# XuyangBai/D3Feat

Measured on NVIDIA H100. Metric: points/sec through KPFCNN encoder, higher is better.
Workload: dtype f32

## Files before the change

### d3feat_b200/csrc/ops.cuh

```cuda
#pragma once
#include "common.cuh"

namespace d3f {

struct Epilogue {
  const float* rowscale;
  const float* bn_scale;
  const float* bn_shift;
  const float* bias;
  const float* residual;
  float leaky_alpha;
  const int* row_map;
  const int* m_dev = nullptr;
  int m_off = 0;
};
int gemm_f32(const float* A, const float* B, float* C, int M, int N, int K, const Epilogue& ep, cudaStream_t stream);

size_t tc_packed_floats(int K, int N);
int tc_padded_n(int N);
int tc_pack_weight(const float* W, int K, int N, float* packed, cudaStream_t stream);
bool tc_gemm_supported(const float* A, int K);
int tc_gemm(const float* A, const float* Bp, float* C, int M, int N, int K, const Epilogue& ep, cudaStream_t stream,
            float* split_ws = nullptr, const float* A2 = nullptr, int K1 = 0);
int tc_gemm_splits(int M, int N, int K);
size_t tc_gemm_split_ws_floats(int M, int N, int K);

int launch_batch_start(const int* len, int B, int* start, cudaStream_t stream);
int bbox_device(const float* pts, int N, float* out_bbox, cudaStream_t stream);
size_t grid_subsample_workspace_bytes(int N, int B);
int grid_subsample(const float* pts, const int* batch_len, int B, int N, float dl, const float* feats, int fdim,
                   const int* classes, int ldim, const float* host_bbox, float* out_pts, float* out_feats,
                   int* out_classes, int* out_batch_len, int* out_M, void* workspace, size_t workspace_bytes,
                   cudaStream_t stream, const int* n_dev = nullptr, int out_capacity = -1, int* status = nullptr,
                   const int* start_pre = nullptr);

size_t voxel_down_sample_workspace_bytes(int N, int B);
int voxel_down_sample(const float* pts, const int* lengths, int B, int N, const int* n_dev, double voxel_size,
                      const float* host_bbox, float* out_pts, int* out_lengths, int* out_M, int out_capacity,
                      int* d_status, void* workspace, size_t workspace_bytes, cudaStream_t stream);

size_t radius_neighbors_workspace_bytes(int Ns, int B, float radius, const float* host_bbox);
int radius_neighbors_build(const float* supports, const int* s_batch_len, int B, int Ns, float radius,
                           const float* host_bbox, void* workspace, size_t workspace_bytes, cudaStream_t stream,
                           const int* ns_dev = nullptr, const int* s_start_pre = nullptr);
int radius_neighbors_count(const float* queries, const int* q_batch_len, int Nq, int B, int Ns, float radius,
                           const float* host_bbox, const void* workspace, int* counts, int* out_max,
                           cudaStream_t stream);
int radius_neighbors_order(const void* workspace, int Ns, int B, float radius, const float* host_bbox, int* out_order,
                           cudaStream_t stream);
int radius_neighbors_fill(const float* queries, const int* q_batch_len, int Nq, int B, int Ns, float radius,
                          const float* host_bbox, const void* workspace, int cols, int pad_value, int* out_idx,
                          cudaStream_t stream, const int* nq_dev = nullptr, const int* pad_dev = nullptr,
                          const int* q_start_pre = nullptr);
struct NbView;
int radius_neighbors_view(const void* workspace, int Ns, int B, float radius, const float* host_bbox, NbView* out);

size_t pyramid_workspace_bytes(int B, const d3f_pyramid_spec* spec, const int* capacity, const float* host_bbox);
int pyramid_build(const float* points, const int* lengths, int B, int N0, const d3f_pyramid_spec* spec,
                  const float* host_bbox, float* const* out_points, int* const* out_lengths,
                  int* const* out_neighbors, int* const* out_pools, int* const* out_upsamples, const int* capacity,
                  int* out_level_sizes, void* workspace, size_t workspace_bytes, cudaStream_t stream,
                  int* d_counts = nullptr, int* d_status = nullptr, const int* n0_dev = nullptr);

size_t kpconv_workspace_bytes(int Nq, int Ns, int H, int K, int Cin, int Cout);
int kpconv_forward_impl(bool deform, const float* q, const float* s, const int* idx, const float* feat,
                        const float* Kp, const float* offsets, const float* modulations, const float* W,
                        const float* W_packed, const int* query_order, int Nq,
                        int Ns, int H, int K, int Cin, int Cout, float extent, int influence, int mode, int normalize,
                        const float* bn_scale, const float* bn_shift, const float* bias, float leaky_alpha,
                        float* out, void* workspace, size_t workspace_bytes, cudaStream_t stream,
                        const int* nq_dev = nullptr, const int* ns_dev = nullptr);

bool kpconv_fused_supported(int Nq, int H, int K, int Cin, int Cout, int influence, int mode, const float* feat,
                            const float* W, const float* out, const int* query_order);
size_t kpconv_fused_workspace_bytes();
int kpconv_fused_forward(const float* q, const float4* s4, const int* idx, const float* feat, const float* Kp,
                         const float* W, float* w_img, int Nq, int Ns, int H, int Cout, float extent, int normalize,
                         const float* bn_scale, const float* bn_shift, const float* bias, float leaky_alpha, float* out,
                         cudaStream_t stream, const int* nq_dev = nullptr, const int* ns_dev = nullptr);

int ind_max_pool(const float* x, const int* inds, int N1, int N2, int H, int C, float* out, void* workspace,
                 size_t workspace_bytes, cudaStream_t stream, const int* n1_dev = nullptr, const int* n2_dev = nullptr);
int closest_pool(const float* x, const int* inds, int N1, int N2, int ld_inds, int C, float* out,
                 cudaStream_t stream, const int* n1_dev = nullptr, const int* n2_dev = nullptr);
int l2_normalize(const float* x, int N, int C, float eps, float* out, cudaStream_t stream, const int* n_dev = nullptr);
size_t detection_scores_workspace_bytes(int N, int B);
int detection_scores(const float* feats, const int* neighbors, const int* lengths, int B, int N, int H, int D,
                     float* out_scores, void* workspace, size_t workspace_bytes, cudaStream_t stream,
                     const int* n_dev = nullptr);
int affine_leaky(const float* x, int N, int C, const float* scale, const float* shift, const float* residual,
                 float alpha, float* out, cudaStream_t stream, const int* n_dev = nullptr);

size_t select_keypoints_workspace_bytes(int N, int B);
int select_keypoints(const float* scores, const int* lengths, int B, int N, int k, const float* points,
                     const float* descriptors, int D, int* out_order, int* out_index, int* out_count, float* out_points,
                     float* out_descriptors, float* out_scores, void* workspace, size_t workspace_bytes,
                     cudaStream_t stream, const int* n_dev = nullptr);

size_t match_descriptors_workspace_bytes(int k, int P);
int match_descriptors(const float* desc, const int* count, int B, int k, int D, const int* pairs, int P, int* nn_st,
                      float* sim_st, int* nn_ts, float* sim_ts, int* matches, int* n_matches, void* workspace,
                      size_t workspace_bytes, cudaStream_t stream);

size_t register_pairs_workspace_bytes(int L, int P, int max_iterations, int max_validation);
int register_pairs(const float* points, const int* count, int B, int k, const int* corr, const int* n_corr, int L,
                   const int* pairs, int P, int ransac_n, int max_iterations, int max_validation, double distance,
                   double edge_ratio, unsigned long long seed, double* pose, int* n_inliers, int* hypothesis,
                   int* n_validated, void* workspace, size_t workspace_bytes, cudaStream_t stream);

size_t icp_pairs_workspace_bytes(int N, int B, int P, double distance, const float* host_bbox);
int icp_pairs(const float* points, const int* lengths, int B, int N, const int* n_dev, const float* host_bbox,
              const int* pairs, int P, const double* init, double distance, int max_iterations,
              double relative_fitness, double relative_rmse, double* pose, double* fitness, double* inlier_rmse,
              int* n_corr, int* iterations, void* workspace, size_t workspace_bytes, cudaStream_t stream);

size_t evaluate_pairs_workspace_bytes(int P, int S);
int evaluate_pairs(const float* points, const int* count, int B, int k, const int* matches, const int* n_matches,
                   int L, const int* pairs, int P, const double* truth_pose, const double* truth_info,
                   const int* truth_flags, const double* const* poses, int S, const int* levels, int R,
                   double fmr_distance, double fmr_ratio, double repeat_distance, double err2, double rte_max,
                   double rre_max_deg, int* valid, int* n_match_inliers, double* inlier_ratio, int* fmr_hit,
                   int* n_repeated, double* repeatability, double* rte, double* rre_deg, double* rmse2, int* success,
                   int* recall_hit, double* totals, void* workspace, size_t workspace_bytes, cudaStream_t stream);

}
```

### d3feat_b200/csrc/tc_common.cuh

```cuda
#pragma once
#include "common.cuh"

namespace d3f {

__device__ __forceinline__ uint32_t smem_u32(const void* p) { return (uint32_t)__cvta_generic_to_shared(p); }

__device__ __forceinline__ void mbar_init(uint32_t bar, uint32_t count) {
  asm volatile("mbarrier.init.shared::cta.b64 [%0], %1;" ::"r"(bar), "r"(count) : "memory");
}
__device__ __forceinline__ void mbar_arrive(uint32_t bar) {
  asm volatile("mbarrier.arrive.shared::cta.b64 _, [%0];" ::"r"(bar) : "memory");
}
__device__ __forceinline__ void mbar_wait(uint32_t bar, uint32_t parity) {
  uint32_t ok;
  do {
    asm volatile(
        "{\n\t.reg .pred p;\n\t"
        "mbarrier.try_wait.parity.shared::cta.b64 p, [%1], %2;\n\t"
        "selp.u32 %0, 1, 0, p;\n\t}"
        : "=r"(ok)
        : "r"(bar), "r"(parity)
        : "memory");
  } while (!ok);
}
__device__ __forceinline__ void fence_proxy_async() { asm volatile("fence.proxy.async.shared::cta;" ::: "memory"); }

__device__ __forceinline__ uint64_t make_smem_desc(uint32_t saddr) {
  uint64_t d = 0;
  d |= (uint64_t)((saddr >> 4) & 0x3FFF);
  d |= (uint64_t)1 << 16;
  d |= (uint64_t)(1024 >> 4) << 32;
  d |= (uint64_t)1 << 62;
  return d;
}

__device__ __forceinline__ void wgmma_fence() { asm volatile("wgmma.fence.sync.aligned;" ::: "memory"); }
__device__ __forceinline__ void wgmma_commit() { asm volatile("wgmma.commit_group.sync.aligned;" ::: "memory"); }
template <int N>
__device__ __forceinline__ void wgmma_wait() { asm volatile("wgmma.wait_group.sync.aligned %0;" ::"n"(N) : "memory"); }
template <int R>
__device__ __forceinline__ void wgmma_reg_fence(float* d) {
#pragma unroll
  for (int i = 0; i < R; ++i) asm volatile("" : "+f"(d[i])::"memory");
}

template <int N>
__device__ __forceinline__ void wgmma_tf32(float* d, uint64_t adesc, uint64_t bdesc);
template <>
__device__ __forceinline__ void wgmma_tf32<32>(float* d, uint64_t adesc, uint64_t bdesc) {
  asm volatile(
      "{\n\t.reg .pred p;\n\tsetp.ne.b32 p, %18, 0;\n\t"
      "wgmma.mma_async.sync.aligned.m64n32k8.f32.tf32.tf32 "
      "{%0, %1, %2, %3, %4, %5, %6, %7, %8, %9, %10, %11, %12, %13, %14, %15}, %16, %17, p, 1, 1;\n\t}"
      : "+f"(d[0]), "+f"(d[1]), "+f"(d[2]), "+f"(d[3]), "+f"(d[4]), "+f"(d[5]), "+f"(d[6]), "+f"(d[7]), "+f"(d[8]), "+f"(d[9]), "+f"(d[10]), "+f"(d[11]), "+f"(d[12]), "+f"(d[13]), "+f"(d[14]), "+f"(d[15])
      : "l"(adesc), "l"(bdesc), "r"(1)
      : "memory");
}
template <>
__device__ __forceinline__ void wgmma_tf32<64>(float* d, uint64_t adesc, uint64_t bdesc) {
  asm volatile(
      "{\n\t.reg .pred p;\n\tsetp.ne.b32 p, %34, 0;\n\t"
      "wgmma.mma_async.sync.aligned.m64n64k8.f32.tf32.tf32 "
      "{%0, %1, %2, %3, %4, %5, %6, %7, %8, %9, %10, %11, %12, %13, %14, %15, %16, %17, %18, %19, %20, %21, %22, %23, %24, %25, %26, %27, %28, %29, %30, %31}, %32, %33, p, 1, 1;\n\t}"
      : "+f"(d[0]), "+f"(d[1]), "+f"(d[2]), "+f"(d[3]), "+f"(d[4]), "+f"(d[5]), "+f"(d[6]), "+f"(d[7]), "+f"(d[8]), "+f"(d[9]), "+f"(d[10]), "+f"(d[11]), "+f"(d[12]), "+f"(d[13]), "+f"(d[14]), "+f"(d[15]), "+f"(d[16]), "+f"(d[17]), "+f"(d[18]), "+f"(d[19]), "+f"(d[20]), "+f"(d[21]), "+f"(d[22]), "+f"(d[23]), "+f"(d[24]), "+f"(d[25]), "+f"(d[26]), "+f"(d[27]), "+f"(d[28]), "+f"(d[29]), "+f"(d[30]), "+f"(d[31])
      : "l"(adesc), "l"(bdesc), "r"(1)
      : "memory");
}
template <>
__device__ __forceinline__ void wgmma_tf32<96>(float* d, uint64_t adesc, uint64_t bdesc) {
  asm volatile(
      "{\n\t.reg .pred p;\n\tsetp.ne.b32 p, %50, 0;\n\t"
      "wgmma.mma_async.sync.aligned.m64n96k8.f32.tf32.tf32 "
      "{%0, %1, %2, %3, %4, %5, %6, %7, %8, %9, %10, %11, %12, %13, %14, %15, %16, %17, %18, %19, %20, %21, %22, %23, %24, %25, %26, %27, %28, %29, %30, %31, %32, %33, %34, %35, %36, %37, %38, %39, %40, %41, %42, %43, %44, %45, %46, %47}, %48, %49, p, 1, 1;\n\t}"
      : "+f"(d[0]), "+f"(d[1]), "+f"(d[2]), "+f"(d[3]), "+f"(d[4]), "+f"(d[5]), "+f"(d[6]), "+f"(d[7]), "+f"(d[8]), "+f"(d[9]), "+f"(d[10]), "+f"(d[11]), "+f"(d[12]), "+f"(d[13]), "+f"(d[14]), "+f"(d[15]), "+f"(d[16]), "+f"(d[17]), "+f"(d[18]), "+f"(d[19]), "+f"(d[20]), "+f"(d[21]), "+f"(d[22]), "+f"(d[23]), "+f"(d[24]), "+f"(d[25]), "+f"(d[26]), "+f"(d[27]), "+f"(d[28]), "+f"(d[29]), "+f"(d[30]), "+f"(d[31]), "+f"(d[32]), "+f"(d[33]), "+f"(d[34]), "+f"(d[35]), "+f"(d[36]), "+f"(d[37]), "+f"(d[38]), "+f"(d[39]), "+f"(d[40]), "+f"(d[41]), "+f"(d[42]), "+f"(d[43]), "+f"(d[44]), "+f"(d[45]), "+f"(d[46]), "+f"(d[47])
      : "l"(adesc), "l"(bdesc), "r"(1)
      : "memory");
}
template <>
__device__ __forceinline__ void wgmma_tf32<128>(float* d, uint64_t adesc, uint64_t bdesc) {
  asm volatile(
      "{\n\t.reg .pred p;\n\tsetp.ne.b32 p, %66, 0;\n\t"
      "wgmma.mma_async.sync.aligned.m64n128k8.f32.tf32.tf32 "
      "{%0, %1, %2, %3, %4, %5, %6, %7, %8, %9, %10, %11, %12, %13, %14, %15, %16, %17, %18, %19, %20, %21, %22, %23, %24, %25, %26, %27, %28, %29, %30, %31, %32, %33, %34, %35, %36, %37, %38, %39, %40, %41, %42, %43, %44, %45, %46, %47, %48, %49, %50, %51, %52, %53, %54, %55, %56, %57, %58, %59, %60, %61, %62, %63}, %64, %65, p, 1, 1;\n\t}"
      : "+f"(d[0]), "+f"(d[1]), "+f"(d[2]), "+f"(d[3]), "+f"(d[4]), "+f"(d[5]), "+f"(d[6]), "+f"(d[7]), "+f"(d[8]), "+f"(d[9]), "+f"(d[10]), "+f"(d[11]), "+f"(d[12]), "+f"(d[13]), "+f"(d[14]), "+f"(d[15]), "+f"(d[16]), "+f"(d[17]), "+f"(d[18]), "+f"(d[19]), "+f"(d[20]), "+f"(d[21]), "+f"(d[22]), "+f"(d[23]), "+f"(d[24]), "+f"(d[25]), "+f"(d[26]), "+f"(d[27]), "+f"(d[28]), "+f"(d[29]), "+f"(d[30]), "+f"(d[31]), "+f"(d[32]), "+f"(d[33]), "+f"(d[34]), "+f"(d[35]), "+f"(d[36]), "+f"(d[37]), "+f"(d[38]), "+f"(d[39]), "+f"(d[40]), "+f"(d[41]), "+f"(d[42]), "+f"(d[43]), "+f"(d[44]), "+f"(d[45]), "+f"(d[46]), "+f"(d[47]), "+f"(d[48]), "+f"(d[49]), "+f"(d[50]), "+f"(d[51]), "+f"(d[52]), "+f"(d[53]), "+f"(d[54]), "+f"(d[55]), "+f"(d[56]), "+f"(d[57]), "+f"(d[58]), "+f"(d[59]), "+f"(d[60]), "+f"(d[61]), "+f"(d[62]), "+f"(d[63])
      : "l"(adesc), "l"(bdesc), "r"(1)
      : "memory");
}

template <int N>
__device__ __forceinline__ void wgmma_tf32_rs(float* d, const uint32_t* a, uint64_t bdesc);
template <>
__device__ __forceinline__ void wgmma_tf32_rs<32>(float* d, const uint32_t* a, uint64_t bdesc) {
  asm volatile(
      "{\n\t.reg .pred p;\n\tsetp.ne.b32 p, %21, 0;\n\t"
      "wgmma.mma_async.sync.aligned.m64n32k8.f32.tf32.tf32 "
      "{%0, %1, %2, %3, %4, %5, %6, %7, %8, %9, %10, %11, %12, %13, %14, %15}, {%16, %17, %18, %19}, %20, p, 1, 1;\n\t}"
      : "+f"(d[0]), "+f"(d[1]), "+f"(d[2]), "+f"(d[3]), "+f"(d[4]), "+f"(d[5]), "+f"(d[6]), "+f"(d[7]), "+f"(d[8]), "+f"(d[9]), "+f"(d[10]), "+f"(d[11]), "+f"(d[12]), "+f"(d[13]), "+f"(d[14]), "+f"(d[15])
      : "r"(a[0]), "r"(a[1]), "r"(a[2]), "r"(a[3]), "l"(bdesc), "r"(1)
      : "memory");
}
template <>
__device__ __forceinline__ void wgmma_tf32_rs<64>(float* d, const uint32_t* a, uint64_t bdesc) {
  asm volatile(
      "{\n\t.reg .pred p;\n\tsetp.ne.b32 p, %37, 0;\n\t"
      "wgmma.mma_async.sync.aligned.m64n64k8.f32.tf32.tf32 "
      "{%0, %1, %2, %3, %4, %5, %6, %7, %8, %9, %10, %11, %12, %13, %14, %15, %16, %17, %18, %19, %20, %21, %22, %23, %24, %25, %26, %27, %28, %29, %30, %31}, {%32, %33, %34, %35}, %36, p, 1, 1;\n\t}"
      : "+f"(d[0]), "+f"(d[1]), "+f"(d[2]), "+f"(d[3]), "+f"(d[4]), "+f"(d[5]), "+f"(d[6]), "+f"(d[7]), "+f"(d[8]), "+f"(d[9]), "+f"(d[10]), "+f"(d[11]), "+f"(d[12]), "+f"(d[13]), "+f"(d[14]), "+f"(d[15]), "+f"(d[16]), "+f"(d[17]), "+f"(d[18]), "+f"(d[19]), "+f"(d[20]), "+f"(d[21]), "+f"(d[22]), "+f"(d[23]), "+f"(d[24]), "+f"(d[25]), "+f"(d[26]), "+f"(d[27]), "+f"(d[28]), "+f"(d[29]), "+f"(d[30]), "+f"(d[31])
      : "r"(a[0]), "r"(a[1]), "r"(a[2]), "r"(a[3]), "l"(bdesc), "r"(1)
      : "memory");
}
template <>
__device__ __forceinline__ void wgmma_tf32_rs<128>(float* d, const uint32_t* a, uint64_t bdesc) {
  asm volatile(
      "{\n\t.reg .pred p;\n\tsetp.ne.b32 p, %69, 0;\n\t"
      "wgmma.mma_async.sync.aligned.m64n128k8.f32.tf32.tf32 "
      "{%0, %1, %2, %3, %4, %5, %6, %7, %8, %9, %10, %11, %12, %13, %14, %15, %16, %17, %18, %19, %20, %21, %22, %23, %24, %25, %26, %27, %28, %29, %30, %31, %32, %33, %34, %35, %36, %37, %38, %39, %40, %41, %42, %43, %44, %45, %46, %47, %48, %49, %50, %51, %52, %53, %54, %55, %56, %57, %58, %59, %60, %61, %62, %63}, {%64, %65, %66, %67}, %68, p, 1, 1;\n\t}"
      : "+f"(d[0]), "+f"(d[1]), "+f"(d[2]), "+f"(d[3]), "+f"(d[4]), "+f"(d[5]), "+f"(d[6]), "+f"(d[7]), "+f"(d[8]), "+f"(d[9]), "+f"(d[10]), "+f"(d[11]), "+f"(d[12]), "+f"(d[13]), "+f"(d[14]), "+f"(d[15]), "+f"(d[16]), "+f"(d[17]), "+f"(d[18]), "+f"(d[19]), "+f"(d[20]), "+f"(d[21]), "+f"(d[22]), "+f"(d[23]), "+f"(d[24]), "+f"(d[25]), "+f"(d[26]), "+f"(d[27]), "+f"(d[28]), "+f"(d[29]), "+f"(d[30]), "+f"(d[31]), "+f"(d[32]), "+f"(d[33]), "+f"(d[34]), "+f"(d[35]), "+f"(d[36]), "+f"(d[37]), "+f"(d[38]), "+f"(d[39]), "+f"(d[40]), "+f"(d[41]), "+f"(d[42]), "+f"(d[43]), "+f"(d[44]), "+f"(d[45]), "+f"(d[46]), "+f"(d[47]), "+f"(d[48]), "+f"(d[49]), "+f"(d[50]), "+f"(d[51]), "+f"(d[52]), "+f"(d[53]), "+f"(d[54]), "+f"(d[55]), "+f"(d[56]), "+f"(d[57]), "+f"(d[58]), "+f"(d[59]), "+f"(d[60]), "+f"(d[61]), "+f"(d[62]), "+f"(d[63])
      : "r"(a[0]), "r"(a[1]), "r"(a[2]), "r"(a[3]), "l"(bdesc), "r"(1)
      : "memory");
}

__device__ __forceinline__ float4 lds128(uint32_t addr) {
  float4 v;
  asm volatile("ld.shared.v4.f32 {%0, %1, %2, %3}, [%4];" : "=f"(v.x), "=f"(v.y), "=f"(v.z), "=f"(v.w) : "r"(addr));
  return v;
}
__device__ __forceinline__ void sts128(uint32_t addr, float4 v) {
  asm volatile("st.shared.v4.f32 [%0], {%1, %2, %3, %4};" ::"r"(addr), "f"(v.x), "f"(v.y), "f"(v.z), "f"(v.w) : "memory");
}
__device__ __forceinline__ void sts64(uint32_t addr, float x, float y) {
  asm volatile("st.shared.v2.f32 [%0], {%1, %2};" ::"r"(addr), "f"(x), "f"(y) : "memory");
}
__device__ __forceinline__ float lds32(uint32_t addr) {
  float v;
  asm volatile("ld.shared.f32 %0, [%1];" : "=f"(v) : "r"(addr));
  return v;
}
__device__ __forceinline__ void sts32(uint32_t addr, float v) {
  asm volatile("st.shared.f32 [%0], %1;" ::"r"(addr), "f"(v) : "memory");
}

__device__ __forceinline__ void split_tf32(float x, float& hi, float& lo) {
  hi = __uint_as_float((__float_as_uint(x) + 0x1000u) & 0xFFFFE000u);
  lo = x - hi;
}

__device__ __forceinline__ void tma_bulk_g2s(uint32_t dst_smem, const void* src, uint32_t bytes, uint32_t bar) {
  asm volatile("cp.async.bulk.shared::cluster.global.mbarrier::complete_tx::bytes [%0], [%1], %2, [%3];"
               ::"r"(dst_smem), "l"(src), "r"(bytes), "r"(bar) : "memory");
}
__device__ __forceinline__ void tma_load_2d(uint32_t dst_smem, const void* tmap, int x, int y, uint32_t bar) {
  asm volatile("cp.async.bulk.tensor.2d.shared::cluster.global.mbarrier::complete_tx::bytes [%0], [%1, {%2, %3}], [%4];"
               ::"r"(dst_smem), "l"(tmap), "r"(x), "r"(y), "r"(bar) : "memory");
}
__device__ __forceinline__ void mbar_arrive_expect_tx(uint32_t bar, uint32_t bytes) {
  asm volatile("mbarrier.arrive.expect_tx.shared::cta.b64 _, [%0], %1;" ::"r"(bar), "r"(bytes) : "memory");
}
__device__ __forceinline__ void cp_async16(uint32_t dst_smem, const void* src) {
  asm volatile("cp.async.cg.shared.global [%0], [%1], 16;" ::"r"(dst_smem), "l"(src) : "memory");
}
__device__ __forceinline__ void cp_async16_zfill(uint32_t dst_smem, const void* src, bool valid) {
  const int sz = valid ? 16 : 0;
  asm volatile("cp.async.cg.shared.global [%0], [%1], 16, %2;" ::"r"(dst_smem), "l"(src), "r"(sz) : "memory");
}

}
```

### d3feat_b200/csrc/tc_gemm.cu

```cuda
#include <cuda.h>
#include <cudaTypedefs.h>
#include <stdlib.h>

#include "ops.cuh"
#include "tc_common.cuh"

namespace d3f {

constexpr int kTcBM = 128;
constexpr int kTcBK = 32;
constexpr int kTcConsumerWarps = 8;
constexpr int kTcThreads = 32 * kTcConsumerWarps + 32;

__global__ void __launch_bounds__(256) pack_weight_kernel(const float* __restrict__ W, int K, int N, int Kpad,
                                                          int Npad, float* __restrict__ packed) {
  long long total = (long long)Npad * Kpad;
  for (long long i = (long long)blockIdx.x * blockDim.x + threadIdx.x; i < total; i += (long long)gridDim.x * blockDim.x) {
    int k = (int)(i / Npad), n = (int)(i % Npad);
    float x = (n < N && k < K) ? W[(size_t)k * N + n] : 0.f;
    float hi, lo;
    split_tf32(x, hi, lo);
    int kc = k >> 5, kl = k & 31;
    size_t slab = (size_t)kc * 2 * Npad * 32;
    size_t off = (size_t)n * 32 + (size_t)((((kl >> 2) ^ (n & 7)) << 2) | (kl & 3));
    packed[slab + off] = hi;
    packed[slab + (size_t)Npad * 32 + off] = lo;
  }
}

int tc_padded_k(int K) { return (K + kTcBK - 1) / kTcBK * kTcBK; }
int tc_block_n(int N) { return N > 64 ? 128 : (N > 32 ? 64 : 32); }
int tc_padded_n(int N) { int bn = tc_block_n(N); return (N + bn - 1) / bn * bn; }
size_t tc_packed_floats(int K, int N) { return 2 * (size_t)tc_padded_k(K) * tc_padded_n(N); }

int tc_pack_weight(const float* W, int K, int N, float* packed, cudaStream_t stream) {
  D3F_REQUIRE(K >= 1 && N >= 1 && W && packed, D3F_ERR_INVALID, "pack_weight: bad arguments");
  int Kpad = tc_padded_k(K), Npad = tc_padded_n(N);
  long long total = (long long)Npad * Kpad;
  int blocks = (int)min((total + 255) / 256, (long long)kNumSMs * 8);
  pack_weight_kernel<<<blocks, 256, 0, stream>>>(W, K, N, Kpad, Npad, packed);
  D3F_LAUNCH_CHECK("pack_weight_kernel");
  return D3F_OK;
}

template <int BN>
struct TcSmem {
  static constexpr int kCtasPerSm = BN >= 128 ? 1 : 2;
  static constexpr int kStages = BN >= 64 ? 3 : 4;
  static constexpr int kABytes = kTcBM * 128;
  static constexpr int kBBytes = BN * 128;
  static constexpr int kStageBytes = kABytes + 2 * kBBytes;
  static constexpr int kEpiWarpBytes = 1024 + 3 * BN * 4;
  static constexpr int kTotal = kStages * kStageBytes + 1024  + 256  + kTcConsumerWarps * kEpiWarpBytes;
  static_assert(kCtasPerSm * (kTotal + 1024) <= 233472, "shared memory of an H100 SM (228 KB, 1 KB reserved per CTA)");
};

template <int BN>
__global__ void __launch_bounds__(kTcThreads, TcSmem<BN>::kCtasPerSm)
tc_gemm_kernel(const __grid_constant__ CUtensorMap tmA, const __grid_constant__ CUtensorMap tmA2, int K1,
               const float* __restrict__ Bp, float* __restrict__ C, int Mcap, int N, int Kpad, int Npad,
               int chunks_per_split, Epilogue ep) {
  const int M = ep.m_dev ? min(Mcap, max(__ldg(ep.m_dev) - ep.m_off, 0)) : Mcap;
  const int ntn = Npad / BN;
  const int tiles = ceil_div(M, kTcBM) * ntn;
  if ((int)blockIdx.x >= tiles) return;
  extern __shared__ uint8_t smem_raw[];
  using S = TcSmem<BN>;
  constexpr int kStages = S::kStages;
  uint8_t* smem = (uint8_t*)(((uintptr_t)smem_raw + 1023) & ~(uintptr_t)1023);
  uint64_t* full = (uint64_t*)(smem + kStages * S::kStageBytes);
  uint64_t* empty = full + kStages;

  const int tid = threadIdx.x, warp = tid >> 5, lane = tid & 31;
  const int kt0 = blockIdx.z * chunks_per_split;
  const int nk = min(Kpad / kTcBK - kt0, chunks_per_split);
  float* Cz = C + (size_t)blockIdx.z * Mcap * N;

  if (tid == 0) {
    for (int s = 0; s < kStages; ++s) {
      mbar_init(smem_u32(&full[s]), 1);
      mbar_init(smem_u32(&empty[s]), kTcConsumerWarps);
    }
    asm volatile("fence.mbarrier_init.release.cluster;" ::: "memory");
  }
  __syncthreads();

  if (warp == kTcConsumerWarps) {
    if (lane == 0) {
      const int total = (tiles - (int)blockIdx.x + (int)gridDim.x - 1) / (int)gridDim.x * nk;
      int tile = (int)blockIdx.x, kt = 0;
      for (int g = 0; g < total; ++g) {
        const int s = g % kStages;
        mbar_wait(smem_u32(&empty[s]), ((uint32_t)(g / kStages) & 1u) ^ 1u);
        const uint32_t st = smem_u32(smem + s * S::kStageBytes);
        const uint32_t fb = smem_u32(&full[s]);
        const int m0 = (tile / ntn) * kTcBM, n0 = (tile % ntn) * BN;
        const int k0 = (kt0 + kt) * kTcBK;
        mbar_arrive_expect_tx(fb, (uint32_t)S::kStageBytes);
        if (k0 < K1)
          tma_load_2d(st, &tmA, k0, m0, fb);
        else
          tma_load_2d(st, &tmA2, k0 - K1, m0, fb);
        const float* slab = Bp + (size_t)(kt0 + kt) * 2 * Npad * 32 + (size_t)n0 * 32;
        tma_bulk_g2s(st + S::kABytes, slab, S::kBBytes, fb);
        tma_bulk_g2s(st + S::kABytes + S::kBBytes, slab + (size_t)Npad * 32, S::kBBytes, fb);
        if (++kt == nk) {
          kt = 0;
          tile += (int)gridDim.x;
        }
      }
    }
  } else {
    constexpr int R = BN / 2;
    const int cw = warp >> 2;
    const int wq = warp & 3;
    const int r0 = 64 * cw + 16 * wq + (lane >> 2);
    const uint32_t a_row = (uint32_t)r0 * 128u + (uint32_t)(lane & 3) * 4u, a_swz = (uint32_t)(r0 & 7);
    auto load_a = [&](float* x, uint32_t sa, int j) {
#pragma unroll
      for (int q = 0; q < 4; ++q)
        x[q] = lds32(sa + a_row + (uint32_t)(q & 1) * 1024u + ((((uint32_t)(2 * j + (q >> 1))) ^ a_swz) << 4));
    };
    float acc[R], sum[R];
    int g = 0;
    for (int t = (int)blockIdx.x; t < tiles; t += (int)gridDim.x) {
      const int m0 = (t / ntn) * kTcBM, n0 = (t % ntn) * BN;
#pragma unroll
      for (int j = 0; j < R; ++j) sum[j] = 0.f;
      for (int kt = 0; kt < nk; ++kt, ++g) {
        const int s = g % kStages;
        mbar_wait(smem_u32(&full[s]), (uint32_t)(g / kStages) & 1u);
        const uint32_t sa = smem_u32(smem + s * S::kStageBytes);
        const uint64_t b_hi = make_smem_desc(sa + S::kABytes), b_lo = make_smem_desc(sa + S::kABytes + S::kBBytes);
        float x[4];
        uint32_t ah[2][4], al[2][4];
        load_a(x, sa, 0);
#pragma unroll
        for (int j = 0; j < R; ++j) acc[j] = 0.f;
#pragma unroll
        for (int j = 0; j < kTcBK / 8; ++j) {
          uint32_t* h = ah[j & 1];
          uint32_t* l = al[j & 1];
#pragma unroll
          for (int q = 0; q < 4; ++q) {
            float hi, lo;
            split_tf32(x[q], hi, lo);
            h[q] = __float_as_uint(hi);
            l[q] = __float_as_uint(lo);
          }
          const uint64_t adv = (uint64_t)((j * 32) >> 4);
          wgmma_fence();
          wgmma_tf32_rs<BN>(acc, h, b_hi + adv);
          wgmma_tf32_rs<BN>(acc, l, b_hi + adv);
          wgmma_tf32_rs<BN>(acc, h, b_lo + adv);
          wgmma_commit();
          if (j + 1 < kTcBK / 8) load_a(x, sa, j + 1);
          wgmma_wait<1>();
        }
        wgmma_wait<0>();
        wgmma_reg_fence<R>(acc);
        __syncwarp();
        if (lane == 0) mbar_arrive(smem_u32(&empty[s]));
#pragma unroll
        for (int j = 0; j < R; ++j) sum[j] += acc[j];
      }
      const bool has_bn = ep.bn_scale != nullptr, has_bias = ep.bias != nullptr, has_res = ep.residual != nullptr;
      const bool has_leaky = ep.leaky_alpha >= 0.f;
      const bool vec = (N & 3) == 0 &&
                       ((reinterpret_cast<uintptr_t>(C) | reinterpret_cast<uintptr_t>(ep.residual)) & 15) == 0;
      const uint32_t st_tile = smem_u32(smem + kStages * S::kStageBytes + 256) + (uint32_t)warp * S::kEpiWarpBytes;
      const uint32_t st_par = st_tile + 1024u;
      if (t == (int)blockIdx.x || ntn > 1) {
        for (int c = lane; c < BN; c += 32) {
          const int n = n0 + c;
          if (has_bn) {
            sts32(st_par + 4u * c, n < N ? ep.bn_scale[n] : 0.f);
            sts32(st_par + 4u * (BN + c), n < N ? ep.bn_shift[n] : 0.f);
          }
          if (has_bias) sts32(st_par + 4u * (2 * BN + c), n < N ? ep.bias[n] : 0.f);
        }
      }
#pragma unroll
      for (int h = 0; h < 2; ++h) {
#pragma unroll
        for (int cg = 0; cg < BN / 32; ++cg) {
          {
            const uint32_t r = (uint32_t)(lane >> 2), tq = (uint32_t)(lane & 3);
            const uint32_t swz = ((r & 3u) << 1) ^ (r >> 2);
#pragma unroll
            for (int jj = 0; jj < 4; ++jj) {
              const int j = 4 * cg + jj;
              sts64(st_tile + r * 128u + (((uint32_t)(2 * jj) + (tq >> 1)) ^ swz) * 16u + (tq & 1u) * 8u,
                    sum[4 * j + 2 * h], sum[4 * j + 2 * h + 1]);
            }
          }
          __syncwarp();
          const int pc = lane & 7;
          const int gn = n0 + 32 * cg + 4 * pc;
          const uint32_t par = st_par + 4u * (32 * cg + 4 * pc);
#pragma unroll
          for (int i = 0; i < 2; ++i) {
            const uint32_t r = (uint32_t)(lane >> 3) + 4u * i;
            const float4 v = lds128(st_tile + r * 128u + (((uint32_t)pc ^ ((r & 3u) << 1) ^ (r >> 2)) << 4));
            const int gm = m0 + 64 * cw + 16 * wq + 8 * h + (int)r;
            if (gm >= M || gn >= N) continue;
            const float rs = ep.rowscale != nullptr ? ep.rowscale[gm] : 1.f;
            const size_t orow = ep.row_map ? (size_t)ep.row_map[gm] : (size_t)gm;
            float* cp = Cz + orow * N + gn;
            const float* rp = has_res ? ep.residual + orow * N + gn : nullptr;
            float y[4] = {v.x * rs, v.y * rs, v.z * rs, v.w * rs};
            float res[4] = {0.f, 0.f, 0.f, 0.f};
            if (has_res) {
              if (vec) {
                const float4 rv = *reinterpret_cast<const float4*>(rp);
                res[0] = rv.x; res[1] = rv.y; res[2] = rv.z; res[3] = rv.w;
              } else {
#pragma unroll
                for (int e = 0; e < 4; ++e)
                  if (gn + e < N) res[e] = rp[e];
              }
            }
            if (has_bn) {
              const float4 sc = lds128(par), sh = lds128(par + 4u * BN);
              y[0] = fmaf(y[0], sc.x, sh.x); y[1] = fmaf(y[1], sc.y, sh.y);
              y[2] = fmaf(y[2], sc.z, sh.z); y[3] = fmaf(y[3], sc.w, sh.w);
            }
            if (has_bias) {
              const float4 bi = lds128(par + 8u * BN);
              y[0] += bi.x; y[1] += bi.y; y[2] += bi.z; y[3] += bi.w;
            }
#pragma unroll
            for (int e = 0; e < 4; ++e) {
              y[e] += res[e];
              if (has_leaky) y[e] = y[e] > 0.f ? y[e] : y[e] * ep.leaky_alpha;
            }
            if (vec) {
              *reinterpret_cast<float4*>(cp) = make_float4(y[0], y[1], y[2], y[3]);
            } else {
#pragma unroll
              for (int e = 0; e < 4; ++e)
                if (gn + e < N) cp[e] = y[e];
            }
          }
          __syncwarp();
        }
      }
    }
  }
}

__global__ void __launch_bounds__(256) splitk_reduce_kernel(const float* __restrict__ part, int splits, int Mcap, int N,
                                                            Epilogue ep, float* __restrict__ C) {
  const int M = ep.m_dev ? min(Mcap, max(__ldg(ep.m_dev) - ep.m_off, 0)) : Mcap;
  const long long slab = (long long)Mcap * N;
  long long total = (long long)M * N;
  for (long long i = (long long)blockIdx.x * blockDim.x + threadIdx.x; i < total; i += (long long)gridDim.x * blockDim.x) {
    int m = (int)(i / N), n = (int)(i % N);
    float y = 0.f;
    for (int z = 0; z < splits; ++z) y += part[(size_t)z * slab + i];
    if (ep.rowscale) y *= ep.rowscale[m];
    if (ep.bn_scale) y = fmaf(y, ep.bn_scale[n], ep.bn_shift[n]);
    if (ep.bias) y += ep.bias[n];
    const size_t orow = ep.row_map ? (size_t)ep.row_map[m] : (size_t)m;
    if (ep.residual) y += ep.residual[orow * N + n];
    if (ep.leaky_alpha >= 0.f) y = y > 0.f ? y : y * ep.leaky_alpha;
    C[orow * N + n] = y;
  }
}

static int encode_a_map(CUtensorMap* map, const float* A, int rows, int cols) {
  static PFN_cuTensorMapEncodeTiled_v12000 encode = nullptr;
  if (encode == nullptr) {
    void* fn = nullptr;
    cudaDriverEntryPointQueryResult q;
    D3F_CUDA(cudaGetDriverEntryPoint("cuTensorMapEncodeTiled", &fn, cudaEnableDefault, &q));
    D3F_REQUIRE(q == cudaDriverEntryPointSuccess && fn != nullptr, D3F_ERR_CUDA,
                "tc_gemm: the driver has no cuTensorMapEncodeTiled");
    encode = reinterpret_cast<PFN_cuTensorMapEncodeTiled_v12000>(fn);
  }
  const cuuint64_t dims[2] = {(cuuint64_t)cols, (cuuint64_t)rows};
  const cuuint64_t strides[1] = {(cuuint64_t)cols * sizeof(float)};
  const cuuint32_t box[2] = {(cuuint32_t)kTcBK, (cuuint32_t)kTcBM};
  const cuuint32_t elem[2] = {1, 1};
  const CUresult r = encode(map, CU_TENSOR_MAP_DATA_TYPE_FLOAT32, 2, const_cast<float*>(A), dims, strides, box, elem,
                            CU_TENSOR_MAP_INTERLEAVE_NONE, CU_TENSOR_MAP_SWIZZLE_128B, CU_TENSOR_MAP_L2_PROMOTION_L2_256B,
                            CU_TENSOR_MAP_FLOAT_OOB_FILL_NONE);
  D3F_REQUIRE(r == CUDA_SUCCESS, D3F_ERR_CUDA, "tc_gemm: cuTensorMapEncodeTiled failed (%d)", (int)r);
  return D3F_OK;
}

template <int BN>
static int launch_tc(const float* A, const float* A2, int K1, const float* Bp, float* C, int M, int N, int K,
                     const Epilogue& ep, cudaStream_t stream, int splits, float* split_ws, bool persistent) {
  using S = TcSmem<BN>;
  static bool configured = false;
  if (!configured) {
    D3F_CUDA(cudaFuncSetAttribute(tc_gemm_kernel<BN>, cudaFuncAttributeMaxDynamicSharedMemorySize, S::kTotal));
    configured = true;
  }
  const int Kpad = tc_padded_k(K), Npad = tc_padded_n(N);
  const int nk = Kpad / kTcBK;
  const int tiles = ceil_div(M, kTcBM) * (Npad / BN);
  CUtensorMap tmA, tmA2;
  if (A2 != nullptr) {
    int rc = encode_a_map(&tmA, A, M, K1);
    if (rc == D3F_OK) rc = encode_a_map(&tmA2, A2, M, K - K1);
    if (rc != D3F_OK) return rc;
  } else {
    const int rc = encode_a_map(&tmA, A, M, K);
    if (rc != D3F_OK) return rc;
    tmA2 = tmA;
    K1 = Kpad;
  }
  if (splits <= 1) {
    const int cap = kNumSMs * S::kCtasPerSm;
    const int grid = persistent && tiles > cap ? cap : tiles;
    tc_gemm_kernel<BN><<<grid, kTcThreads, S::kTotal, stream>>>(tmA, tmA2, K1, Bp, C, M, N, Kpad, Npad, nk, ep);
    D3F_LAUNCH_CHECK("tc_gemm_kernel");
    return D3F_OK;
  }
  const int cps = ceil_div(nk, splits);
  splits = ceil_div(nk, cps);
  Epilogue raw;
  raw.rowscale = nullptr; raw.bn_scale = nullptr; raw.bn_shift = nullptr; raw.bias = nullptr; raw.residual = nullptr;
  raw.leaky_alpha = -1.f; raw.row_map = nullptr; raw.m_dev = ep.m_dev; raw.m_off = ep.m_off;
  dim3 grid(tiles, 1, splits);
  tc_gemm_kernel<BN><<<grid, kTcThreads, S::kTotal, stream>>>(tmA, tmA2, K1, Bp, split_ws, M, N, Kpad, Npad, cps, raw);
  D3F_LAUNCH_CHECK("tc_gemm_kernel");
  long long total = (long long)M * N;
  int blocks = (int)min((total + 255) / 256, (long long)kNumSMs * 8);
  splitk_reduce_kernel<<<blocks, 256, 0, stream>>>(split_ws, splits, M, N, ep, C);
  D3F_LAUNCH_CHECK("splitk_reduce_kernel");
  return D3F_OK;
}

static int env_int(const char* name, int dflt) {
  const char* v = getenv(name);
  return v ? atoi(v) : dflt;
}

bool tc_gemm_supported(const float* A, int K) {
  return (K % 4 == 0) && ((reinterpret_cast<uintptr_t>(A) & 15) == 0);
}

int tc_gemm_splits(int M, int N, int K) {
  const int bn = tc_block_n(N);
  const long long ctas = (long long)ceil_div(M, kTcBM) * (tc_padded_n(N) / bn);
  const int nk = tc_padded_k(K) / kTcBK;
  if (ctas >= 96 || nk < 16) return 1;
  int best = 1;
  long long best_cost = (long long)ceil_div((int)ctas, kNumSMs) * nk * 8;
  for (int s = 2; s <= 8 && s <= nk / 4; ++s) {
    const int cps = ceil_div(nk, s);
    const int eff = ceil_div(nk, cps);
    if (eff != s) continue;
    long long cost = (long long)ceil_div((int)(ctas * s), kNumSMs) * cps * 8 + 40 + 6 * s;
    if (cost < best_cost) {
      best_cost = cost;
      best = s;
    }
  }
  return best;
}
size_t tc_gemm_split_ws_floats(int M, int N, int K) {
  const int bn = tc_block_n(N);
  const long long ctas = (long long)ceil_div(M, kTcBM) * (tc_padded_n(N) / bn);
  const int nk = tc_padded_k(K) / kTcBK;
  if (nk < 16) return 0;
  const long long tiles = ctas < 95 ? ctas : 95;
  return (size_t)(8 * tiles * kTcBM * bn);
}

int tc_gemm(const float* A, const float* Bp, float* C, int M, int N, int K, const Epilogue& ep, cudaStream_t stream,
            float* split_ws, const float* A2, int K1) {
  if (M <= 0 || N <= 0) return D3F_OK;
  D3F_REQUIRE(tc_gemm_supported(A, K), D3F_ERR_INVALID, "tc_gemm: needs K %% 4 == 0 and 16-byte aligned A");
  if (A2 != nullptr)
    D3F_REQUIRE(K1 > 0 && K1 < K && K1 % kTcBK == 0 && tc_gemm_supported(A2, K - K1), D3F_ERR_INVALID,
                "tc_gemm: split A operand needs K1 %% %d == 0 and a 16-byte aligned second matrix", kTcBK);
  int bn = tc_block_n(N);
  if (bn == 128 && K <= 256 && M >= 8192) bn = 64;
  const int splits = split_ws != nullptr ? tc_gemm_splits(M, N, K) : 1;
  const bool persistent = splits <= 1 && (tc_padded_k(K) / kTcBK <= 4 || env_int("D3F_TC_STREAM", 0) != 0);
  switch (bn) {
    case 128: return launch_tc<128>(A, A2, K1, Bp, C, M, N, K, ep, stream, splits, split_ws, persistent);
    case 64: return launch_tc<64>(A, A2, K1, Bp, C, M, N, K, ep, stream, splits, split_ws, persistent);
    default: return launch_tc<32>(A, A2, K1, Bp, C, M, N, K, ep, stream, splits, split_ws, persistent);
  }
}

}
```

Before: 64.66 million.

## Overlap WGMMA chunks with double accumulators and rebalance registers via setmaxnreg

For BN=128 tiles the TF32 tensor-core GEMM now ping-pongs between two accumulator sets, so each K-chunk's accumulation into the running sum and its stage release overlap with the next chunk's wgmma. The producer warpgroup is widened to 128 threads so setmaxnreg can give consumers 240 registers. The epilogue preloads residual, rowscale and row_map before the shared-memory transpose. A cost-model planner may also switch wide-N GEMMs to BN=64 tiles. This trades more registers and idle producer threads for less serialization between chunks.

```diff
diff --git a/d3feat_b200/csrc/ops.cuh b/d3feat_b200/csrc/ops.cuh
--- a/d3feat_b200/csrc/ops.cuh
+++ b/d3feat_b200/csrc/ops.cuh
@@ -22,7 +22,6 @@
 bool tc_gemm_supported(const float* A, int K);
 int tc_gemm(const float* A, const float* Bp, float* C, int M, int N, int K, const Epilogue& ep, cudaStream_t stream,
             float* split_ws = nullptr, const float* A2 = nullptr, int K1 = 0);
-int tc_gemm_splits(int M, int N, int K);
 size_t tc_gemm_split_ws_floats(int M, int N, int K);
 
 int launch_batch_start(const int* len, int B, int* start, cudaStream_t stream);
diff --git a/d3feat_b200/csrc/tc_common.cuh b/d3feat_b200/csrc/tc_common.cuh
--- a/d3feat_b200/csrc/tc_common.cuh
+++ b/d3feat_b200/csrc/tc_common.cuh
@@ -38,6 +38,10 @@
 __device__ __forceinline__ void wgmma_commit() { asm volatile("wgmma.commit_group.sync.aligned;" ::: "memory"); }
 template <int N>
 __device__ __forceinline__ void wgmma_wait() { asm volatile("wgmma.wait_group.sync.aligned %0;" ::"n"(N) : "memory"); }
+template <int N>
+__device__ __forceinline__ void setmaxnreg_dec() { asm volatile("setmaxnreg.dec.sync.aligned.u32 %0;" ::"n"(N)); }
+template <int N>
+__device__ __forceinline__ void setmaxnreg_inc() { asm volatile("setmaxnreg.inc.sync.aligned.u32 %0;" ::"n"(N)); }
 template <int R>
 __device__ __forceinline__ void wgmma_reg_fence(float* d) {
 #pragma unroll
diff --git a/d3feat_b200/csrc/tc_gemm.cu b/d3feat_b200/csrc/tc_gemm.cu
--- a/d3feat_b200/csrc/tc_gemm.cu
+++ b/d3feat_b200/csrc/tc_gemm.cu
@@ -10,7 +10,6 @@
 constexpr int kTcBM = 128;
 constexpr int kTcBK = 32;
 constexpr int kTcConsumerWarps = 8;
-constexpr int kTcThreads = 32 * kTcConsumerWarps + 32;
 
 __global__ void __launch_bounds__(256) pack_weight_kernel(const float* __restrict__ W, int K, int N, int Kpad,
                                                           int Npad, float* __restrict__ packed) {
@@ -46,6 +45,10 @@
 template <int BN>
 struct TcSmem {
   static constexpr int kCtasPerSm = BN >= 128 ? 1 : 2;
+  static constexpr bool kOverlap = BN >= 128;
+  static constexpr int kThreads = 32 * kTcConsumerWarps + (kOverlap ? 128 : 32);
+  static constexpr int kProducerRegs = 24, kConsumerRegs = 240;
+  static_assert(!kOverlap || 128 * kProducerRegs + 256 * kConsumerRegs <= 65536 / kCtasPerSm, "register file");
   static constexpr int kStages = BN >= 64 ? 3 : 4;
   static constexpr int kABytes = kTcBM * 128;
   static constexpr int kBBytes = BN * 128;
@@ -56,7 +59,7 @@
 };
 
 template <int BN>
-__global__ void __launch_bounds__(kTcThreads, TcSmem<BN>::kCtasPerSm)
+__global__ void __launch_bounds__(TcSmem<BN>::kThreads, TcSmem<BN>::kCtasPerSm)
 tc_gemm_kernel(const __grid_constant__ CUtensorMap tmA, const __grid_constant__ CUtensorMap tmA2, int K1,
                const float* __restrict__ Bp, float* __restrict__ C, int Mcap, int N, int Kpad, int Npad,
                int chunks_per_split, Epilogue ep) {
@@ -85,8 +88,9 @@
   }
   __syncthreads();
 
-  if (warp == kTcConsumerWarps) {
-    if (lane == 0) {
+  if (warp >= kTcConsumerWarps) {
+    if constexpr (S::kOverlap) setmaxnreg_dec<S::kProducerRegs>();
+    if (warp == kTcConsumerWarps && lane == 0) {
       const int total = (tiles - (int)blockIdx.x + (int)gridDim.x - 1) / (int)gridDim.x * nk;
       int tile = (int)blockIdx.x, kt = 0;
       for (int g = 0; g < total; ++g) {
@@ -111,6 +115,7 @@
       }
     }
   } else {
+    if constexpr (S::kOverlap) setmaxnreg_inc<S::kConsumerRegs>();
     constexpr int R = BN / 2;
     const int cw = warp >> 2;
     const int wq = warp & 3;
@@ -121,49 +126,73 @@
       for (int q = 0; q < 4; ++q)
         x[q] = lds32(sa + a_row + (uint32_t)(q & 1) * 1024u + ((((uint32_t)(2 * j + (q >> 1))) ^ a_swz) << 4));
     };
-    float acc[R], sum[R];
+    float acc[R], acc2[S::kOverlap ? R : 1], sum[R];
+    float x[4];
+    uint32_t ah[2][4], al[2][4];
+    auto run_chunk = [&](float* a, const float* prev, int gg, bool add_prev) {
+      const int s = gg % kStages;
+      mbar_wait(smem_u32(&full[s]), (uint32_t)(gg / kStages) & 1u);
+      const uint32_t sa = smem_u32(smem + s * S::kStageBytes);
+      const uint64_t b_hi = make_smem_desc(sa + S::kABytes), b_lo = make_smem_desc(sa + S::kABytes + S::kBBytes);
+      load_a(x, sa, 0);
+#pragma unroll
+      for (int j = 0; j < R; ++j) a[j] = 0.f;
+#pragma unroll
+      for (int j = 0; j < kTcBK / 8; ++j) {
+        uint32_t* h = ah[j & 1];
+        uint32_t* l = al[j & 1];
+#pragma unroll
+        for (int q = 0; q < 4; ++q) {
+          float hi, lo;
+          split_tf32(x[q], hi, lo);
+          h[q] = __float_as_uint(hi);
+          l[q] = __float_as_uint(lo);
+        }
+        const uint64_t adv = (uint64_t)((j * 32) >> 4);
+        wgmma_fence();
+        wgmma_tf32_rs<BN>(a, h, b_hi + adv);
+        wgmma_tf32_rs<BN>(a, l, b_hi + adv);
+        wgmma_tf32_rs<BN>(a, h, b_lo + adv);
+        wgmma_commit();
+        if (j + 1 < kTcBK / 8) load_a(x, sa, j + 1);
+        wgmma_wait<1>();
+        if (add_prev && j == 0) {
+          wgmma_reg_fence<R>(const_cast<float*>(prev));
+          __syncwarp();
+          if (lane == 0) mbar_arrive(smem_u32(&empty[(gg - 1) % kStages]));
+#pragma unroll
+          for (int i = 0; i < R; ++i) sum[i] += prev[i];
+        }
+      }
+    };
+    auto drain = [&](float* a, int gg) {
+      wgmma_wait<0>();
+      wgmma_reg_fence<R>(a);
+      __syncwarp();
+      if (lane == 0) mbar_arrive(smem_u32(&empty[gg % kStages]));
+#pragma unroll
+      for (int i = 0; i < R; ++i) sum[i] += a[i];
+    };
     int g = 0;
     for (int t = (int)blockIdx.x; t < tiles; t += (int)gridDim.x) {
       const int m0 = (t / ntn) * kTcBM, n0 = (t % ntn) * BN;
 #pragma unroll
       for (int j = 0; j < R; ++j) sum[j] = 0.f;
-      for (int kt = 0; kt < nk; ++kt, ++g) {
-        const int s = g % kStages;
-        mbar_wait(smem_u32(&full[s]), (uint32_t)(g / kStages) & 1u);
-        const uint32_t sa = smem_u32(smem + s * S::kStageBytes);
-        const uint64_t b_hi = make_smem_desc(sa + S::kABytes), b_lo = make_smem_desc(sa + S::kABytes + S::kBBytes);
-        float x[4];
-        uint32_t ah[2][4], al[2][4];
-        load_a(x, sa, 0);
-#pragma unroll
-        for (int j = 0; j < R; ++j) acc[j] = 0.f;
-#pragma unroll
-        for (int j = 0; j < kTcBK / 8; ++j) {
-          uint32_t* h = ah[j & 1];
-          uint32_t* l = al[j & 1];
-#pragma unroll
-          for (int q = 0; q < 4; ++q) {
-            float hi, lo;
-            split_tf32(x[q], hi, lo);
-            h[q] = __float_as_uint(hi);
-            l[q] = __float_as_uint(lo);
-          }
-          const uint64_t adv = (uint64_t)((j * 32) >> 4);
-          wgmma_fence();
-          wgmma_tf32_rs<BN>(acc, h, b_hi + adv);
-          wgmma_tf32_rs<BN>(acc, l, b_hi + adv);
-          wgmma_tf32_rs<BN>(acc, h, b_lo + adv);
-          wgmma_commit();
-          if (j + 1 < kTcBK / 8) load_a(x, sa, j + 1);
-          wgmma_wait<1>();
-        }
-        wgmma_wait<0>();
-        wgmma_reg_fence<R>(acc);
-        __syncwarp();
-        if (lane == 0) mbar_arrive(smem_u32(&empty[s]));
-#pragma unroll
-        for (int j = 0; j < R; ++j) sum[j] += acc[j];
-      }
+      int kt = 0;
+      if constexpr (S::kOverlap) {
+        for (; kt + 4 <= nk; kt += 4) {
+          run_chunk(acc, acc2, g + kt, false);
+          run_chunk(acc2, acc, g + kt + 1, true);
+          run_chunk(acc, acc2, g + kt + 2, true);
+          run_chunk(acc2, acc, g + kt + 3, true);
+          drain(acc2, g + kt + 3);
+        }
+      }
+      for (; kt < nk; ++kt) {
+        run_chunk(acc, acc, g + kt, false);
+        drain(acc, g + kt);
+      }
+      g += nk;
       const bool has_bn = ep.bn_scale != nullptr, has_bias = ep.bias != nullptr, has_res = ep.residual != nullptr;
       const bool has_leaky = ep.leaky_alpha >= 0.f;
       const bool vec = (N & 3) == 0 &&
@@ -180,8 +209,27 @@
           if (has_bias) sts32(st_par + 4u * (2 * BN + c), n < N ? ep.bias[n] : 0.f);
         }
       }
+      const int pc = lane & 7;
 #pragma unroll
       for (int h = 0; h < 2; ++h) {
+        float rs[2];
+        size_t orow[2];
+        bool row_ok[2];
+        float4 rv[BN / 32][2];
+#pragma unroll
+        for (int i = 0; i < 2; ++i) {
+          const int gm = m0 + 64 * cw + 16 * wq + 8 * h + (lane >> 3) + 4 * i;
+          row_ok[i] = gm < M;
+          rs[i] = row_ok[i] && ep.rowscale != nullptr ? ep.rowscale[gm] : 1.f;
+          orow[i] = row_ok[i] && ep.row_map ? (size_t)ep.row_map[gm] : (size_t)gm;
+#pragma unroll
+          for (int cg = 0; cg < BN / 32; ++cg) {
+            const int gn = n0 + 32 * cg + 4 * pc;
+            rv[cg][i] = make_float4(0.f, 0.f, 0.f, 0.f);
+            if (has_res && vec && row_ok[i] && gn < N)
+              rv[cg][i] = *reinterpret_cast<const float4*>(ep.residual + orow[i] * N + gn);
+          }
+        }
 #pragma unroll
         for (int cg = 0; cg < BN / 32; ++cg) {
           {
@@ -195,30 +243,21 @@
             }
           }
           __syncwarp();
-          const int pc = lane & 7;
           const int gn = n0 + 32 * cg + 4 * pc;
           const uint32_t par = st_par + 4u * (32 * cg + 4 * pc);
 #pragma unroll
           for (int i = 0; i < 2; ++i) {
             const uint32_t r = (uint32_t)(lane >> 3) + 4u * i;
             const float4 v = lds128(st_tile + r * 128u + (((uint32_t)pc ^ ((r & 3u) << 1) ^ (r >> 2)) << 4));
-            const int gm = m0 + 64 * cw + 16 * wq + 8 * h + (int)r;
-            if (gm >= M || gn >= N) continue;
-            const float rs = ep.rowscale != nullptr ? ep.rowscale[gm] : 1.f;
-            const size_t orow = ep.row_map ? (size_t)ep.row_map[gm] : (size_t)gm;
-            float* cp = Cz + orow * N + gn;
-            const float* rp = has_res ? ep.residual + orow * N + gn : nullptr;
-            float y[4] = {v.x * rs, v.y * rs, v.z * rs, v.w * rs};
-            float res[4] = {0.f, 0.f, 0.f, 0.f};
-            if (has_res) {
-              if (vec) {
-                const float4 rv = *reinterpret_cast<const float4*>(rp);
-                res[0] = rv.x; res[1] = rv.y; res[2] = rv.z; res[3] = rv.w;
-              } else {
-#pragma unroll
-                for (int e = 0; e < 4; ++e)
-                  if (gn + e < N) res[e] = rp[e];
-              }
+            if (!row_ok[i] || gn >= N) continue;
+            float* cp = Cz + orow[i] * N + gn;
+            float y[4] = {v.x * rs[i], v.y * rs[i], v.z * rs[i], v.w * rs[i]};
+            float res[4] = {rv[cg][i].x, rv[cg][i].y, rv[cg][i].z, rv[cg][i].w};
+            if (has_res && !vec) {
+              const float* rp = ep.residual + orow[i] * N + gn;
+#pragma unroll
+              for (int e = 0; e < 4; ++e)
+                if (gn + e < N) res[e] = rp[e];
             }
             if (has_bn) {
               const float4 sc = lds128(par), sh = lds128(par + 4u * BN);
@@ -315,7 +354,7 @@
   if (splits <= 1) {
     const int cap = kNumSMs * S::kCtasPerSm;
     const int grid = persistent && tiles > cap ? cap : tiles;
-    tc_gemm_kernel<BN><<<grid, kTcThreads, S::kTotal, stream>>>(tmA, tmA2, K1, Bp, C, M, N, Kpad, Npad, nk, ep);
+    tc_gemm_kernel<BN><<<grid, S::kThreads, S::kTotal, stream>>>(tmA, tmA2, K1, Bp, C, M, N, Kpad, Npad, nk, ep);
     D3F_LAUNCH_CHECK("tc_gemm_kernel");
     return D3F_OK;
   }
@@ -325,7 +364,7 @@
   raw.rowscale = nullptr; raw.bn_scale = nullptr; raw.bn_shift = nullptr; raw.bias = nullptr; raw.residual = nullptr;
   raw.leaky_alpha = -1.f; raw.row_map = nullptr; raw.m_dev = ep.m_dev; raw.m_off = ep.m_off;
   dim3 grid(tiles, 1, splits);
-  tc_gemm_kernel<BN><<<grid, kTcThreads, S::kTotal, stream>>>(tmA, tmA2, K1, Bp, split_ws, M, N, Kpad, Npad, cps, raw);
+  tc_gemm_kernel<BN><<<grid, S::kThreads, S::kTotal, stream>>>(tmA, tmA2, K1, Bp, split_ws, M, N, Kpad, Npad, cps, raw);
   D3F_LAUNCH_CHECK("tc_gemm_kernel");
   long long total = (long long)M * N;
   int blocks = (int)min((total + 255) / 256, (long long)kNumSMs * 8);
@@ -343,7 +382,7 @@
   return (K % 4 == 0) && ((reinterpret_cast<uintptr_t>(A) & 15) == 0);
 }
 
-int tc_gemm_splits(int M, int N, int K) {
+static int tc_gemm_splits(int M, int N, int K) {
   const int bn = tc_block_n(N);
   const long long ctas = (long long)ceil_div(M, kTcBM) * (tc_padded_n(N) / bn);
   const int nk = tc_padded_k(K) / kTcBK;
@@ -362,6 +401,32 @@
   }
   return best;
 }
+
+constexpr float kChunkUs128 = 1.005f, kChunkUs64 = 0.801f, kChunkUs64Pair = 1.561f;
+
+static float tc_wave_us(long long ctas, int bn, int cps) {
+  const long long per_sm = (ctas + kNumSMs - 1) / kNumSMs;
+  if (bn >= 128) return (float)per_sm * cps * kChunkUs128;
+  return per_sm <= 1 ? cps * kChunkUs64 : (float)((per_sm + 1) / 2) * cps * kChunkUs64Pair;
+}
+
+struct TcPlan {
+  int bn, splits;
+  bool persistent;
+};
+static TcPlan tc_gemm_plan(int M, int N, int K, bool has_ws) {
+  const int nk = tc_padded_k(K) / kTcBK;
+  TcPlan p;
+  p.bn = tc_block_n(N);
+  if (p.bn == 128 && K <= 256 && M >= 8192) p.bn = 64;
+  p.splits = has_ws ? tc_gemm_splits(M, N, K) : 1;
+  if (p.bn == 128 && p.splits <= 1 && N > 128) {
+    const long long rows = ceil_div(M, kTcBM), npad = tc_padded_n(N);
+    if (tc_wave_us(rows * (npad / 64), 64, nk) < tc_wave_us(rows * (npad / 128), 128, nk)) p.bn = 64;
+  }
+  p.persistent = p.splits <= 1 && (nk <= 4 || env_int("D3F_TC_STREAM", 0) != 0);
+  return p;
+}
 size_t tc_gemm_split_ws_floats(int M, int N, int K) {
   const int bn = tc_block_n(N);
   const long long ctas = (long long)ceil_div(M, kTcBM) * (tc_padded_n(N) / bn);
@@ -378,11 +443,10 @@
   if (A2 != nullptr)
     D3F_REQUIRE(K1 > 0 && K1 < K && K1 % kTcBK == 0 && tc_gemm_supported(A2, K - K1), D3F_ERR_INVALID,
                 "tc_gemm: split A operand needs K1 %% %d == 0 and a 16-byte aligned second matrix", kTcBK);
-  int bn = tc_block_n(N);
-  if (bn == 128 && K <= 256 && M >= 8192) bn = 64;
-  const int splits = split_ws != nullptr ? tc_gemm_splits(M, N, K) : 1;
-  const bool persistent = splits <= 1 && (tc_padded_k(K) / kTcBK <= 4 || env_int("D3F_TC_STREAM", 0) != 0);
-  switch (bn) {
+  const TcPlan plan = tc_gemm_plan(M, N, K, split_ws != nullptr);
+  const int splits = plan.splits;
+  const bool persistent = plan.persistent;
+  switch (plan.bn) {
     case 128: return launch_tc<128>(A, A2, K1, Bp, C, M, N, K, ep, stream, splits, split_ws, persistent);
     case 64: return launch_tc<64>(A, A2, K1, Bp, C, M, N, K, ep, stream, splits, split_ws, persistent);
     default: return launch_tc<32>(A, A2, K1, Bp, C, M, N, K, ep, stream, splits, split_ws, persistent);
```

Measured after the change: 65.68 million, median of 6. +1.6%, better.
